# RocketFlash/EmbeddingNet

Hardware: AMD Instinct MI355X
Metric: images/sec training (ResNet18, 224², triplet batch-hard) @ 1/2/4/8 GPU (higher is better)
Workload: dtype f32; 1 GPU; resnet18 224x224x3 synthetic U[0,1), 107-class P x K sampling, local batch 32x4=128 (139 resident batches cycled), E=256, margin 0.5, mining 'hardest' per local batch, radam, fp32 tensors (conv products on 16-bit MFMA from operand splits, fp32 accumulate: 3x3 stride-1 convs and their weight gradients, and the ResNets' other convs where both operands' ranges are known: two fp16 pieces + a per-tenso; global_batch=128, parallelism=dp1, active_triplets_min=192, dead_steps=0, resident_batches=139, step_mode=eager, mining=hardest

## Files before the change

embeddingnet_amd/csrc/conv.hip:

```cpp
#include "gemm_engine.h"
#include "conv_geom.h"
#include "../../include/embnet.h"
#include <stdlib.h>

namespace embnet {

struct InputTransform { const float* scale; const float* shift; int act; };
__device__ __forceinline__ float4 transform4(float4 v, bool ok, const float4& sc, const float4& sh, int act) {
  float4 z = make_float4(fmaf(v.x, sc.x, sh.x), fmaf(v.y, sc.y, sh.y), fmaf(v.z, sc.z, sh.z), fmaf(v.w, sc.w, sh.w));
  if (act == 1) {
    z = make_float4(fmaxf(z.x, 0.f), fmaxf(z.y, 0.f), fmaxf(z.z, 0.f), fmaxf(z.w, 0.f));
  } else if (act == 2) {
    z = make_float4(act_apply(2, z.x), act_apply(2, z.y), act_apply(2, z.z), act_apply(2, z.w));
  }
  return ok ? z : make_float4(0.f, 0.f, 0.f, 0.f);
}


template <int ROWS, bool VEC, bool TF = false>
struct LoadConvFwdA {
  using Tile = TileKC<ROWS>;
  static constexpr bool CAN_INTERLEAVE = VEC && !TF;
  Buf buf; int H, W, C, Kg; FastDiv dC, dS; int tid;
  unsigned base[Tile::PASSES]; int ih0[Tile::PASSES], iw0[Tile::PASSES];
// ... 356 lines not shown
        d.x += o.x; d.y += o.y; d.z += o.z; d.w += o.w;
      }
      const float4 o = red[2][threadIdx.x + s * qpb];
      float4& d = red[2][threadIdx.x];
      d.x = fmaxf(d.x, o.x); d.y = fmaxf(d.y, o.y); d.z = fmaxf(d.z, o.z); d.w = fmaxf(d.w, o.w);
    }
    __syncthreads();
  }
  if (rr == 0 && col < cols) {
    const long prow = (long)(tile / tiles_n) * (bm / wtm) + band, P = stats_rows;
    const float4 s1 = red[0][threadIdx.x], s2 = red[1][threadIdx.x];
    float* d1 = stats + (long)col * P + prow;
    float* d2 = d1 + (long)cols * P;
    d1[0] = s1.x; d1[P] = s1.y; d1[2 * P] = s1.z; d1[3 * P] = s1.w;
    d2[0] = s2.x; d2[P] = s2.y; d2[2 * P] = s2.z; d2[3 * P] = s2.w;
    if (bsum.x && bsum.kinds == 3) {
      const float4 s3 = red[2][threadIdx.x];
      float* d3 = d2 + (long)cols * P;
      d3[0] = s3.x; d3[P] = s3.y; d3[2 * P] = s3.z; d3[3 * P] = s3.w;
    }
  }
}

template <class G, bool VEC, bool TF, bool H = false>
__device__ __forceinline__ void conv_fwd_body(const ConvFwdParams& p) {
  using TA = TileKC<G::BM>;
  using TB = TileKM<G::BN>;
  __shared__ __attribute__((aligned(16))) float smem[SMEM_FLOATS<G, TA, TB>];
  prio_hi();
  const int M = p.g.N * p.g.OH * p.g.OW, Kg = p.g.R * p.g.S * p.g.C;
  const int tiles_n = (p.g.K + G::BN - 1) / G::BN;
  int id, k0, k1; float* part;
  tail_decode<G>(p.tail, blockIdx.x, (Kg + BK - 1) / BK, id, k0, k1, part);
  const int m0 = (id / tiles_n) * G::BM, n0 = (id % tiles_n) * G::BN;
  stamp(0);
  LoadConvFwdA<G::BM, VEC, TF> la; la.init(p.x, p.g, m0, threadIdx.x, p.tf);
  LoadRowsKM<G::BN, VEC> lb; lb.init(p.w, p.g.K, p.g.K, Kg, n0, threadIdx.x);
  f32x16 acc[G::TM][G::TN];
  stamp(2);
  if constexpr (H) {
    const float2 sa = range_scale(p.rg.a), sb = range_scale(p.rg.b);
    conv_mainloop<G, TA, TB, decltype(la), decltype(lb), true>(la, lb, k0, k1, smem, acc, (int)blockIdx.x >= p.fair_from, true, sa.x, sb.x);
    scale_acc<G>(acc, sa.y, sb.y);
  } else {
    conv_mainloop<G, TA, TB>(la, lb, k0, k1, smem, acc, (int)blockIdx.x >= p.fair_from);
  }
  stamp(4);
  if (part) { store_partial<G>(acc, smem, part); stamp(5); return; }
  if (VEC) {
    float4 s1 = make_float4(0.f, 0.f, 0.f, 0.f), s2 = s1;
    constexpr int NJ = EpiIdx<G>::NJ;
    const int ecol = n0 + epi_col<G>();
    const bool cok = ecol < p.g.K;
    float4 bv = make_float4(0.f, 0.f, 0.f, 0.f);
    if (p.bias && cok) bv = *reinterpret_cast<const float4*>(p.bias + ecol);
    float4 res[G::TM][NJ];
    if (p.residual) {
#pragma unroll
      for (int im = 0; im < G::TM; ++im)
#pragma unroll
        for (int j = 0; j < NJ; ++j)
          res[im][j] = *reinterpret_cast<const float4*>(p.residual + (long)min(m0 + epi_row<G>(im, j), M - 1) * p.g.K + (cok ? ecol : 0));
// ... 33 lines not shown
      }
    }
    stamp(5);
    return;
  }
  for_each_acc<G>(acc, [&](int r, int c, float v) {
    const int row = m0 + r, col = n0 + c;
    if (row < M && col < p.g.K) {
      if (p.bias) v += p.bias[col];
      if (p.relu) v = fmaxf(v, 0.f);
      if (p.residual) v += p.residual[(long)row * p.g.K + col];
      p.y[(long)row * p.g.K + col] = v;
    }
  });
}

template <class G, bool VEC>
__global__ __launch_bounds__(256, VEC ? CONV_OCC<G> : 1) void conv_fwd_kernel(ConvFwdParams p) { conv_fwd_body<G, VEC, false>(p); }
template <class G, bool VEC>
__global__ __launch_bounds__(256, CONV_OCC<G>) void conv_fwd_tf_kernel(ConvFwdParams p) { conv_fwd_body<G, true, true>(p); }
template <class G>
__global__ __launch_bounds__(256, CONV_OCC_H<G>) void conv_fwd_h_kernel(ConvFwdParams p) { conv_fwd_body<G, true, false, true>(p); }

struct ConvDgradParams { const float* dy; const float* w; float* dx; ConvGeom g; DgradClass cls[MAX_CLASSES]; SplitTail tail; int accumulate; const float* add_src; int fair_from; BnSums bn; Ranges rg; };

template <class G, bool VEC, bool H = false>
__device__ __forceinline__ void conv_dgrad_body(const ConvDgradParams& p) {
  using TA = TileKC<G::BM>;
  using TB = TileKC<G::BN>;
  __shared__ __attribute__((aligned(16))) float smem[SMEM_FLOATS<G, TA, TB>];
  prio_hi();
  const DgradClass& cg = p.cls[blockIdx.y];
  const int M = p.g.N * cg.Hc * cg.Wc, Kg = cg.nR * cg.nS * p.g.K;
  const int tiles_n = (p.g.C + G::BN - 1) / G::BN;
  int id, k0, k1; float* part;
  tail_decode<G>(p.tail, blockIdx.x, (Kg + BK - 1) / BK, id, k0, k1, part);
  const int m0 = (id / tiles_n) * G::BM, n0 = (id % tiles_n) * G::BN;
  if (m0 >= M) return;
  if (Kg == 0 && p.accumulate && p.add_src == p.dx) return;
  stamp(0);
  LoadConvDgradA<G::BM, VEC> la; la.init(p.dy, p.g, cg, m0, threadIdx.x);
  LoadConvDgradB<G::BN, VEC> lb; lb.init(p.w, p.g, cg, n0, threadIdx.x);
  f32x16 acc[G::TM][G::TN];
  stamp(2);
  if constexpr (H) {
    const float2 sa = range_scale(p.rg.a), sb = range_scale(p.rg.b);
    conv_mainloop<G, TA, TB, decltype(la), decltype(lb), true>(la, lb, k0, k1, smem, acc, (int)(blockIdx.y * gridDim.x + blockIdx.x) >= p.fair_from,
                                                               true, sa.x, sb.x);
    scale_acc<G>(acc, sa.y, sb.y);
  } else {
    conv_mainloop<G, TA, TB>(la, lb, k0, k1, smem, acc, (int)(blockIdx.y * gridDim.x + blockIdx.x) >= p.fair_from);
  }
  stamp(4);
  if (part) { store_partial<G>(acc, smem, part); stamp(5); return; }
  const int st = p.g.stride;
  if ((p.g.C & 3) == 0) {
    constexpr int NJ = EpiIdx<G>::NJ;
    const int ecol = n0 + epi_col<G>();
    const bool cok = ecol < p.g.C;
    long base[G::TM][NJ];
    float4 res[G::TM][NJ];
    const bool bnon = p.bn.x != nullptr;
    const float* pre = bnon ? p.bn.x : p.add_src;
#pragma unroll
    for (int im = 0; im < G::TM; ++im)
#pragma unroll
      for (int j = 0; j < NJ; ++j) {
        uint32_t n, rem, hc, wc;
        cg.dHWc.divmod((uint32_t)min(m0 + epi_row<G>(im, j), M - 1), n, rem); cg.dWc.divmod(rem, hc, wc);
        base[im][j] = (((long)n * p.g.H + cg.hoff + st * (int)hc) * p.g.W + cg.woff + st * (int)wc) * p.g.C;
        if (p.accumulate || bnon) res[im][j] = *reinterpret_cast<const float4*>(pre + base[im][j] + (cok ? ecol : 0));
      }
// ... 38 lines not shown
          d3[0] = s3.x; d3[P] = s3.y; d3[2 * P] = s3.z; d3[3 * P] = s3.w;
        }
      }
    }
    stamp(5);
    return;
  }
  int last_r = -1; long row_base = 0;
  for_each_acc<G>(acc, [&](int r, int c, float v) {
    const int row = m0 + r, col = n0 + c;
    if (r != last_r) {
      last_r = r;
      uint32_t n, rem, hc, wc;
      cg.dHWc.divmod((uint32_t)min(row, M - 1), n, rem); cg.dWc.divmod(rem, hc, wc);
      row_base = (((long)n * p.g.H + cg.hoff + st * (int)hc) * p.g.W + cg.woff + st * (int)wc) * p.g.C;
    }
    if (row < M && col < p.g.C) p.dx[row_base + col] = p.accumulate ? p.add_src[row_base + col] + v : v;
  });
}
template <class G, bool VEC>
__global__ __launch_bounds__(256, VEC ? CONV_OCC<G> : 1) void conv_dgrad_kernel(ConvDgradParams p) { conv_dgrad_body<G, VEC>(p); }
template <class G>
__global__ __launch_bounds__(256, CONV_OCC_H<G>) void conv_dgrad_h_kernel(ConvDgradParams p) { conv_dgrad_body<G, true, true>(p); }

struct ConvWgradParams { const float* x; const float* dy; float* out; ConvGeom g; int kt_per_split, splits; InputTransform tf; int fair_from; Ranges rg; };

template <class G, bool VA, bool VB, bool TF, bool H = false>
__device__ __forceinline__ void conv_wgrad_body(const ConvWgradParams& p) {
  using TA = TileKM<G::BM>;
  using TB = TileKM<G::BN>;
  __shared__ __attribute__((aligned(16))) float smem[SMEM_FLOATS<G, TA, TB>];
  prio_hi();
  const int M = p.g.R * p.g.S * p.g.C, Kg = p.g.N * p.g.OH * p.g.OW;
  const int tiles_n = (p.g.K + G::BN - 1) / G::BN;
  const int tiles = ((M + G::BM - 1) / G::BM) * tiles_n;
  const int split = blockIdx.x / tiles, tile = blockIdx.x % tiles;
  if (split >= p.splits) return;
  const int m0 = (tile / tiles_n) * G::BM, n0 = (tile % tiles_n) * G::BN;
  const int kt_total = (Kg + BK - 1) / BK;
  const int kt0 = split * p.kt_per_split, kt1 = min(kt0 + p.kt_per_split, kt_total);
  stamp(0);
  LoadConvWgradA<G::BM, VA, TF> la; la.init(p.x, p.g, m0, threadIdx.x, p.tf);
  LoadRowsKM<G::BN, VB> lb; lb.init(p.dy, p.g.K, p.g.K, Kg, n0, threadIdx.x);
  f32x16 acc[G::TM][G::TN];
  stamp(2);
  if constexpr (H) {
// ... 296 lines not shown

extern "C" size_t embnet_conv2d_fwd_workspace_bytes(int n, int c, int r, int s, int k, int oh, int ow) {
  if (n <= 0 || c <= 0 || r <= 0 || s <= 0 || k <= 0 || oh <= 0 || ow <= 0 || ((c | k) & 3)) return 0;
  const long M = (long)n * oh * ow;
  const int tile = pick_tile(M, k, false, (long)r * s * c);
  SplitTail t; size_t need;
  plan_tail((long)cdiv(M, TILE_BM[tile]) * cdiv(k, TILE_BN[tile]), cdiv((long)r * s * c, BK), TILE_BM[tile], TILE_BN[tile],
            0, t, &need);
  return need;
}

extern "C" int embnet_conv2d_fwd_stats_rows(int n, int c, int r, int s, int k, int oh, int ow) {
  if (n <= 0 || c <= 0 || r <= 0 || s <= 0 || k <= 0 || oh <= 0 || ow <= 0 || ((c | k) & 3)) return 0;
  const long M = (long)n * oh * ow;
  if (r == 1 && s == 1 && thin_gemm_applies(c, k)) return thin_gemm_stats_rows(M, k);
  const int tile = pick_tile(M, k, false, (long)r * s * c);
  return cdiv(M, TILE_BM[tile]) * (TILE_BM[tile] / TILE_WTM[tile]);
}

static int conv2d_fwd_impl(const float* x, const float* w, const float* bias, float* y, int n, int h,
                           int wd, int c, int r, int s, int k, int stride, int pad_t, int pad_l, int oh,
                           int ow, int relu, const float* residual, const float* in_scale,
                           const float* in_shift, int in_act, float* stats, void* workspace,
                           size_t workspace_bytes, void* stream, const Ranges rg) {
  const bool ranged = ranges_ok(rg);
  EMBNET_CHECK_ARG(x && w && y, "conv2d_fwd: null pointer");
  EMBNET_CHECK_ARG(!in_scale == !in_shift, "conv2d_fwd: in_scale and in_shift go together");
  EMBNET_CHECK_ARG(aligned16(y) && aligned16(workspace) && aligned16(residual),
                   "conv2d_fwd: output, residual and workspace must be 16-byte aligned");
  ConvFwdParams p{x, w, bias, y, {}, relu, {}, residual};
  if (int rc = make_geom(p.g, n, h, wd, c, r, s, k, stride, pad_t, pad_l, oh, ow, "conv2d_fwd")) return rc;
  const long M = (long)n * oh * ow;
  hipStream_t st = (hipStream_t)stream;
  if (r == 1 && s == 1 && thin_gemm_applies(c, k)) {
    const bool can = pad_t == 0 && pad_l == 0 && !in_scale && aligned16(x) && aligned16(w) && aligned16(bias) && aligned16(stats);
    if (can) return launch_thin_gemm(x, w, 0, M, c, k, y, stats, bias, relu, residual, stride, n, h, wd, oh, ow, st);
    EMBNET_CHECK_ARG(!stats, "conv2d_fwd: epilogue statistics of a thin 1x1 conv go with pad 0 and no input transform");
  }
  const bool vec = (c & 3) == 0 && (k & 3) == 0 && aligned16(x) && aligned16(w) && (!bias || aligned16(bias));
  const bool hform = ranged && vec && !in_scale;
  const int tile = pick_tile(M, k, false, (long)r * s * c);
  const long tiles = (long)cdiv(M, TILE_BM[tile]) * cdiv(k, TILE_BN[tile]);
  EMBNET_CHECK_ARG(!in_scale || (vec && aligned16(in_scale) && aligned16(in_shift)),
                   "conv2d_fwd: the fused input transform needs channel counts that are multiples of 4 and aligned pointers");
  EMBNET_CHECK_ARG(!stats || (vec && aligned16(stats)),
                   "conv2d_fwd: epilogue statistics need channel counts that are multiples of 4 (see conv2d_fwd_stats_rows)");
  p.tf = InputTransform{in_scale, in_shift, in_act};
  p.stats = stats;
  p.stats_rows = cdiv(M, TILE_BM[tile]) * (TILE_BM[tile] / TILE_WTM[tile]);
  plan_tail(tiles, cdiv((long)r * s * c, BK), TILE_BM[tile], TILE_BN[tile], (vec && workspace) ? workspace_bytes : 0, p.tail);
  p.tail.ws = (float*)workspace;
  const int grid = p.tail.n_full + (int)(tiles - p.tail.n_full) * p.tail.parts;
  p.fair_from = fair_from(grid, tile, false);
  const double flop = 2.0 * M * k * r * s * c;
  p.rg = rg;
  {
    EMBNET_TRACE_FLOP(hform ? conv_h_kernel_name("conv_fwd_h_kernel", "ConvFwdParams", tile) :
                      conv_kernel_name(in_scale ? "conv_fwd_tf_kernel" : "conv_fwd_kernel", "ConvFwdParams", tile,
                                       (vec || in_scale) ? "true" : "false"), flop,
                      4.0 * ((double)n * h * wd * c + (double)r * s * c * k + (double)M * k * (residual ? 2 : 1)), st);
    if (hform) for_tile<false>(tile, [&](auto g) { conv_fwd_h_kernel<decltype(g)><<<grid, 256, 0, st>>>(p); });
    else if (in_scale) for_tile<false>(tile, [&](auto g) { conv_fwd_tf_kernel<decltype(g), true><<<grid, 256, 0, st>>>(p); });
    else if (vec) for_tile<false>(tile, [&](auto g) { conv_fwd_kernel<decltype(g), true><<<grid, 256, 0, st>>>(p); });
    else for_tile<false>(tile, [&](auto g) { conv_fwd_kernel<decltype(g), false><<<grid, 256, 0, st>>>(p); });
  }
  if (p.tail.parts > 1)
    launch_tail_fixup(p.tail.ws, p.tail.parts, TILE_BM[tile], TILE_BN[tile], TILE_WTM[tile], p.tail.n_full, (int)(tiles - p.tail.n_full),
                      cdiv(k, TILE_BN[tile]), M, k, bias, relu, residual, y, stats, p.stats_rows, NO_BN_SUMS, st);
  return check_launch("conv2d_fwd");
}
extern "C" int embnet_conv2d_fwd_f32(const float* x, const float* w, const float* bias, float* y, int n, int h,
                                     int wd, int c, int r, int s, int k, int stride, int pad_t, int pad_l, int oh,
                                     int ow, int relu, const float* residual, const float* in_scale,
                                     const float* in_shift, int in_act, float* stats, void* workspace,
                                     size_t workspace_bytes, void* stream) {
  return conv2d_fwd_impl(x, w, bias, y, n, h, wd, c, r, s, k, stride, pad_t, pad_l, oh, ow, relu, residual, in_scale, in_shift, in_act,
                         stats, workspace, workspace_bytes, stream, take_ranges());
}
extern "C" int embnet_conv2d_fwd_f32_ex(const float* x, const float* w, const float* bias, float* y, int n, int h,
                                        int wd, int c, int r, int s, int k, int stride, int pad_t, int pad_l, int oh,
                                        int ow, int relu, const float* residual, const float* in_scale,
                                        const float* in_shift, int in_act, float* stats, void* workspace,
                                        size_t workspace_bytes, const uint32_t* x_range, const uint32_t* w_range, void* stream) {
  (void)take_ranges();
  return conv2d_fwd_impl(x, w, bias, y, n, h, wd, c, r, s, k, stride, pad_t, pad_l, oh, ow, relu, residual, in_scale, in_shift, in_act,
                         stats, workspace, workspace_bytes, stream, Ranges{x_range, w_range});
}

extern "C" size_t embnet_conv2d_dgrad_workspace_bytes(int n, int h, int wd, int c, int r, int s, int k, int stride) {
  if (n <= 0 || h <= 0 || wd <= 0 || c <= 0 || r <= 0 || s <= 0 || k <= 0 || stride != 1 || ((c | k) & 3)) return 0;
  const long M = (long)n * h * wd;
  const int tile = pick_tile(M, c, false, (long)r * s * k);
  SplitTail t; size_t need;
  plan_tail((long)cdiv(M, TILE_BM[tile]) * cdiv(c, TILE_BN[tile]), cdiv((long)r * s * k, BK), TILE_BM[tile], TILE_BN[tile],
            0, t, &need);
  return need;
}

static int conv2d_dgrad_impl(const float* dy, const float* w, float* dx, int n, int h, int wd, int c,
                             int r, int s, int k, int stride, int pad_t, int pad_l, int oh, int ow,
                             int accumulate, const float* dx_add, void* workspace, size_t workspace_bytes,
                             void* stream, const BnSums bn, const Ranges rg) {
  const bool ranged = ranges_ok(rg);
  EMBNET_CHECK_ARG(dy && w && dx, "conv2d_dgrad: null pointer");
  EMBNET_CHECK_ARG(aligned16(dx) && aligned16(workspace), "conv2d_dgrad: output and workspace must be 16-byte aligned");
  EMBNET_CHECK_ARG(!(accumulate && dx_add), "conv2d_dgrad: accumulate (into dx) or dx_add (another tensor), not both");
  EMBNET_CHECK_ARG(aligned16(dx_add), "conv2d_dgrad: dx_add must be 16-byte aligned");
  ConvDgradParams p{dy, w, dx, {}, {}, {}, (accumulate != 0 || dx_add) ? 1 : 0, dx_add ? dx_add : dx};
  p.bn = bn;
  if (int rc = make_geom(p.g, n, h, wd, c, r, s, k, stride, pad_t, pad_l, oh, ow, "conv2d_dgrad")) return rc;
  if (r == 1 && s == 1 && stride == 1 && pad_t == 0 && pad_l == 0 && !accumulate && !dx_add && !bn.partial && aligned16(dy) &&
      aligned16(w) && thin_gemm_applies(k, c))
    return launch_thin_gemm(dy, w, 1, (long)n * h * wd, k, c, dx, nullptr, nullptr, 0, nullptr, 1, n, h, wd, h, wd, (hipStream_t)stream);
  EMBNET_CHECK_ARG(stride * stride <= MAX_CLASSES, "conv2d_dgrad: stride %d > 3 unsupported", stride);
  long max_m = 0;
  for (int ph = 0; ph < stride; ++ph)
    for (int pw = 0; pw < stride; ++pw) {
      DgradClass& cg = p.cls[ph * stride + pw];
      cg.r0 = ph; cg.s0 = pw;
      cg.hoff = ((ph - pad_t) % stride + stride) % stride; cg.woff = ((pw - pad_l) % stride + stride) % stride;
      cg.Hc = cg.hoff < h ? (h - cg.hoff + stride - 1) / stride : 0;
      cg.Wc = cg.woff < wd ? (wd - cg.woff + stride - 1) / stride : 0;
      cg.nR = ph < r ? (r - ph + stride - 1) / stride : 0;
      cg.nS = pw < s ? (s - pw + stride - 1) / stride : 0;
      cg.hb = (cg.hoff + pad_t - ph) / stride; cg.wb = (cg.woff + pad_l - pw) / stride;
      cg.dHWc = FastDiv::make(cg.Hc * cg.Wc > 0 ? cg.Hc * cg.Wc : 1);
      cg.dWc = FastDiv::make(cg.Wc > 0 ? cg.Wc : 1);
      cg.dnS = FastDiv::make(cg.nS > 0 ? cg.nS : 1);
      const long m = (long)n * cg.Hc * cg.Wc;
      if (m > max_m) max_m = m;
    }
  hipStream_t st = (hipStream_t)stream;
  const int tile = pick_tile(max_m * stride * stride, c, stride > 1, (long)r * s * k);
  const long tiles = (long)cdiv(max_m, TILE_BM[tile]) * cdiv(c, TILE_BN[tile]);
  const bool vec = (k & 3) == 0 && aligned16(dy) && aligned16(w);
  const bool can_split = vec && stride == 1 && (c & 3) == 0 && workspace;
  plan_tail(tiles, cdiv((long)p.cls[0].nR * p.cls[0].nS * k, BK), TILE_BM[tile], TILE_BN[tile],
            can_split ? workspace_bytes : 0, p.tail);
  p.tail.ws = (float*)workspace;
  const dim3 grid(p.tail.n_full + (int)(tiles - p.tail.n_full) * p.tail.parts, stride * stride);
  p.fair_from = fair_from((long)grid.x * grid.y, tile, false);
  const bool hform = ranged && vec;
  p.rg = rg;
  {
    EMBNET_TRACE_FLOP(hform ? conv_h_kernel_name("conv_dgrad_h_kernel", "ConvDgradParams", tile) :
                      conv_kernel_name("conv_dgrad_kernel", "ConvDgradParams", tile, vec ? "true" : "false"),
                      2.0 * n * oh * ow * (double)k * r * s * c,
                      4.0 * ((double)n * oh * ow * k + (double)r * s * c * k + (double)n * h * wd * c * (p.accumulate ? 2 : 1)), st);
    if (hform) for_tile<false>(tile, [&](auto g) { conv_dgrad_h_kernel<decltype(g)><<<grid, 256, 0, st>>>(p); });
    else if (vec) for_tile<false>(tile, [&](auto g) { conv_dgrad_kernel<decltype(g), true><<<grid, 256, 0, st>>>(p); });
    else for_tile<false>(tile, [&](auto g) { conv_dgrad_kernel<decltype(g), false><<<grid, 256, 0, st>>>(p); });
  }
  if (p.tail.parts > 1)
    launch_tail_fixup(p.tail.ws, p.tail.parts, TILE_BM[tile], TILE_BN[tile], TILE_WTM[tile], p.tail.n_full, (int)(tiles - p.tail.n_full),
                      cdiv(c, TILE_BN[tile]), max_m, c, nullptr, 0, p.accumulate ? p.add_src : nullptr, dx, nullptr, 0, p.bn, st);
  return check_launch("conv2d_dgrad");
}

extern "C" int embnet_conv2d_dgrad_f32(const float* dy, const float* w, float* dx, int n, int h, int wd, int c,
                                       int r, int s, int k, int stride, int pad_t, int pad_l, int oh, int ow,
                                       int accumulate, const float* dx_add, void* workspace, size_t workspace_bytes,
                                       void* stream) {
  return conv2d_dgrad_impl(dy, w, dx, n, h, wd, c, r, s, k, stride, pad_t, pad_l, oh, ow, accumulate, dx_add, workspace,
                           workspace_bytes, stream, NO_BN_SUMS, take_ranges());
}
extern "C" int embnet_conv2d_dgrad_f32_ex(const float* dy, const float* w, float* dx, int n, int h, int wd, int c,
                                          int r, int s, int k, int stride, int pad_t, int pad_l, int oh, int ow,
                                          int accumulate, const float* dx_add, void* workspace, size_t workspace_bytes,
                                          const uint32_t* dy_range, const uint32_t* w_range, void* stream) {
  (void)take_ranges();
  return conv2d_dgrad_impl(dy, w, dx, n, h, wd, c, r, s, k, stride, pad_t, pad_l, oh, ow, accumulate, dx_add, workspace,
                           workspace_bytes, stream, NO_BN_SUMS, Ranges{dy_range, w_range});
}

extern "C" int embnet_conv2d_dgrad_bnsums_rows(int n, int h, int wd, int c, int r, int s, int k, int stride) {
  if (n <= 0 || h <= 0 || wd <= 0 || c <= 0 || r <= 0 || s <= 0 || k <= 0 || stride != 1 || ((c | k) & 3)) return 0;
  const long M = (long)n * h * wd;
  const int tile = pick_tile(M, c, false, (long)r * s * k);
  return cdiv(M, TILE_BM[tile]) * (TILE_BM[tile] / TILE_WTM[tile]);
// ... 10 lines not shown
  EMBNET_CHECK_ARG(aligned16(bn_x) && aligned16(bn_scale) && aligned16(bn_shift) && aligned16(bn_mean) && aligned16(bn_rstd) &&
                   aligned16(dy) && aligned16(w), "conv2d_dgrad_bnsums: operands must be 16-byte aligned");
  EMBNET_CHECK_ARG(bn_act >= 0 && bn_act <= 2, "conv2d_dgrad_bnsums: activation code %d", bn_act);
  return conv2d_dgrad_impl(dy, w, dx, n, h, wd, c, r, s, k, stride, pad_t, pad_l, oh, ow, 0, nullptr, workspace, workspace_bytes,
                           stream, BnSums{bn_x, bn_scale, bn_shift, bn_mean, bn_rstd, bn_act, bn_partial, bn_rows, kinds}, rg);
}
extern "C" int embnet_conv2d_dgrad_bnsums_f32(const float* dy, const float* w, float* dx, int n, int h, int wd, int c, int r,
                                              int s, int k, int stride, int pad_t, int pad_l, int oh, int ow,
                                              const float* bn_x, const float* bn_scale, const float* bn_shift,
                                              const float* bn_mean, const float* bn_rstd, int bn_act, float* bn_partial,
                                              int bn_rows, void* workspace, size_t workspace_bytes, void* stream) {
  return conv2d_dgrad_bnsums_impl(dy, w, dx, n, h, wd, c, r, s, k, stride, pad_t, pad_l, oh, ow, bn_x, bn_scale, bn_shift, bn_mean,
                                  bn_rstd, bn_act, bn_partial, bn_rows, workspace, workspace_bytes, stream, take_ranges());
}
extern "C" int embnet_conv2d_dgrad_bnsums_f32_ex(const float* dy, const float* w, float* dx, int n, int h, int wd, int c, int r,
                                                 int s, int k, int stride, int pad_t, int pad_l, int oh, int ow,
                                                 const float* bn_x, const float* bn_scale, const float* bn_shift,
                                                 const float* bn_mean, const float* bn_rstd, int bn_act, float* bn_partial,
                                                 int bn_rows, void* workspace, size_t workspace_bytes,
                                                 const uint32_t* dy_range, const uint32_t* w_range, void* stream) {
  (void)take_ranges();
  return conv2d_dgrad_bnsums_impl(dy, w, dx, n, h, wd, c, r, s, k, stride, pad_t, pad_l, oh, ow, bn_x, bn_scale, bn_shift, bn_mean,
                                  bn_rstd, bn_act, bn_partial, bn_rows, workspace, workspace_bytes, stream, Ranges{dy_range, w_range}, 3);
}

static void wgrad_plan(int rows, int k, long kg, int& tile, int& splits, int& kt_per_split, bool one_by_one = false) {
  if (one_by_one && thin_wgrad_applies(rows, k)) {
    tile = -1; splits = thin_wgrad_splits(kg, rows, k); kt_per_split = 0;
    return;
  }
  tile = (rows <= 64 && k > 32) ? 3 : (k <= 32 ? 2 : (k <= 64 ? 1 : 0));
  if (tile == 1 && rows % 192 == 0 && rows % 128 != 0) tile = 4;
  const int forced_tile = (int)env_long("EMBNET_WGRAD_TILE", -1);
  if (forced_tile >= 0) tile = forced_tile;
  const long tiles = (long)cdiv(rows, TILE_BM[tile]) * cdiv(k, TILE_BN[tile]);
  const int kt_total = cdiv(kg, BK);
#if EMBNET_CONV_SPLIT
  long target = tiles >= 100 ? 1024 : (tiles <= 2 ? 768 : 512);
#else
  long target = tiles >= 100 ? 2048 : (tiles >= 30 ? 1536 : 768);
#endif
  const long forced_blocks = env_long("EMBNET_WGRAD_BLOCKS", 0);
  if (forced_blocks > 0) target = forced_blocks;
#if EMBNET_CONV_SPLIT
  long want = target / tiles;
#else
// ... 122 lines not shown
                                       size_t workspace_bytes, int n, int h, int wd, int c, int r, int s, int k,
                                       int stride, int pad_t, int pad_l, int oh, int ow, const float* in_scale, const float* in_shift, int in_act,
        const uint32_t* x_range, const uint32_t* dy_range, void* stream) {
  (void)take_ranges();
  return wgrad_impl(x, dy, dw, workspace, workspace_bytes, n, h, wd, c, r, s, k, stride, pad_t, pad_l, oh, ow, in_scale, in_shift, in_act,
                    stream, true, false, Ranges{x_range, dy_range});
}
extern "C" int embnet_conv2d_wgrad_reduce_f32(const float* x, const float* dy, float* dw, void* workspace,
                                       size_t workspace_bytes, int n, int h, int wd, int c, int r, int s, int k,
                                       int stride, int pad_t, int pad_l, int oh, int ow, const float* in_scale, const float* in_shift, int in_act,
        void* stream) {
  return wgrad_impl(x, dy, dw, workspace, workspace_bytes, n, h, wd, c, r, s, k, stride, pad_t, pad_l, oh, ow, in_scale, in_shift, in_act,
                    stream, false, true, take_ranges());
}

extern "C" const char* embnet_conv2d_kernel_name(int kind, int n, int h, int wd, int c, int r, int s, int k,
                                                 int oh, int ow) {
  if (kind == 0)
    return conv_kernel_name("conv_fwd_kernel", "ConvFwdParams", pick_tile((long)n * oh * ow, k, false, (long)r * s * c),
                            ((c | k) & 3) == 0 ? "true" : "false");
  if (kind == 1)
    return conv_kernel_name("conv_dgrad_kernel", "ConvDgradParams", pick_tile((long)n * h * wd, c, oh < h, (long)r * s * k),
                            (k & 3) == 0 ? "true" : "false");
  if (kind != 2) return "";
  int tile, sp, kt;
  wgrad_plan(r * s * c, k, (long)n * oh * ow, tile, sp, kt, r == 1 && s == 1);
  if (tile < 0) return "embnet::thinw::thin_wgrad_kernel";
  return conv_kernel_name("conv_wgrad_kernel", "ConvWgradParams", tile,
                          (k & 3) ? "false, false" : ((c & 3) ? "false, true" : "true, true"));
}
```

embeddingnet_amd/layers.py:

```python
import contextlib
import math
import os as _os

import torch
from torch import nn

from . import _lib
from ._lib import check, ptr, stream


def env_switch(var, default):
    return {"0": False, "1": True}.get(_os.environ.get(var), default)


@contextlib.contextmanager
def switches(**values):
    old = {name: globals()[name][0] for name in values}
    try:
        for name, v in values.items():
            globals()[name][0] = v
        yield
    finally:
        for name, v in old.items():
            globals()[name][0] = v
# ... 658 lines not shown
                        _rptr(dy_range), _rptr(w_range) if dy_range is not None else None, stream()))
                    BN_SUMS.put(dx.data_ptr(), (partial, rows, bn_x.data_ptr(), dx.detach()), 8, "oldest")
                else:
                    _gather_dgrad(lib, dz, w, dx, n, h, wd, c, r, s, k, stride, pt, pl, oh, ow, dy_range, w_range, 0, dskip)
        if need_dw:
            conv_wgrad(lib, x, dz, dw, w, n, h, wd, c, r, s, k, stride, pt, pl, oh, ow, in_scale, in_shift, ctx.in_act,
                       ctx.x_planes, dy_planes, dy_range, ctx.x_range)
            dw = _done(dw, dw_note)
        if want_db:
            db, db_note = _sink(ctx.bias_ref)
            _colsum(dz.view(-1, k), out=db)
            db = _done(db, db_note)
        if dskip is not None and dx is None and ctx.needs_input_grad[0]:
            dx = dskip
        if ctx.has_res and dy_only_planes:
            raise _lib.EmbnetError("conv2d backward: a conv with a fused Add received its gradient as planes only; the Add's other "
                                   "branch needs the fp32 gradient (BatchNormalization(owns_input=True) behind conv(residual=...))")
        return dx, dw, db, None, None, (dy if ctx.has_res else None), None, None, None, None, None, None, None, None, None


class _ConvPairFn(torch.autograd.Function):

    @staticmethod
    def forward(ctx, x, w1, geom1, w2, geom2, in_stats, in_act, out_stats1, planes=None, w_ranges=None, x_range=None):
        w_ranges = tuple(w_ranges) if (w_ranges is not None and in_stats is None and x_range is not None) else (None, None)
        x, w1, w2 = _c(x), _c(w1), _c(w2)
        lib = _lib.lib()
        n, h, wd, c = x.shape
        in_scale, in_shift = _in_affine(in_stats)
        ys = []
        for w, geom, st in ((w1, geom1, out_stats1), (w2, geom2, None)):
            r, s, c2, k = w.shape
            if c2 != c:
                raise _lib.EmbnetError(f"conv2d: input has {c} channels, kernel expects {c2}")
            stride, pt, pl, oh, ow = geom
            y = torch.empty((n, oh, ow, k), device=x.device, dtype=torch.float32)
            if planes is not None and w is w1:
                ws = workspace(lib.embnet_conv2d_patch_workspace_bytes(n, c, r, s, k, oh, ow), x.device)
                check(lib.embnet_conv2d_patch_f32(ptr(planes), ptr(weight_planes(w, 0)), None, ptr(y), n, h, wd, c, r, s, k,
                                                  pt, pl, oh, ow, 0, None, ptr(st), ptr(ws), ws.numel() * 4, stream()))
            else:
                _gather_fwd(lib, x, w, None, y, n, h, wd, c, r, s, k, stride, pt, pl, oh, ow, x_range, w_ranges[0 if w is w1 else 1],
                            st, 0, None, in_scale, in_shift, in_act)
            ys.append(y)
        ctx.patch = planes is not None
        ctx.w_ranges = (w_ranges[0] if planes is None else None, w_ranges[1])
        ctx.x_range = x_range
        ctx.x_planes = planes
        ctx.geoms, ctx.in_act = (geom1, geom2), int(in_act)
        ctx.save_for_backward(x, w1, w2, in_stats)
        return ys[0], ys[1]

    @staticmethod
    def backward(ctx, dy1, dy2):
        x, w1, w2, in_stats = ctx.saved_tensors
        lib = _lib.lib()
        n, h, wd, c = x.shape
        in_scale, in_shift = _in_affine(in_stats)
        dx = torch.empty_like(x) if ctx.needs_input_grad[0] else None
        dws, first = [], True
        for w, geom, dy, need_dw in ((w1, ctx.geoms[0], dy1, ctx.needs_input_grad[1]),
                                     (w2, ctx.geoms[1], dy2, ctx.needs_input_grad[3])):
            if dy is None:
                dws.append(None)
                continue
            if not _is_placeholder(dy):
                dy = _c(dy)
            r, s, _, k = w.shape
            stride, pt, pl, oh, ow = geom
            dy_planes = _take_dy_planes(dy) if (ctx.patch and w is w1) else None
            if _is_placeholder(dy) and dy_planes is None:
                raise _lib.EmbnetError("conv_pair backward: the gradient exists only as planes and they are gone (DY_PLANES)")
            w_range = ctx.w_ranges[0 if w is w1 else 1]
            dy_range = _take_dy_range(dy) if (w_range is not None and not _is_placeholder(dy)) else None
            if dx is not None:
                if dy_planes is not None and first and patch_ok(n, oh, ow, k, r, s, c, 1, h, wd):
                    _patch_dgrad(dy_planes, w, dx, n, h, wd, c, r, s, k, pt, pl, oh, ow, None)
                else:
                    _gather_dgrad(lib, dy, w, dx, n, h, wd, c, r, s, k, stride, pt, pl, oh, ow, dy_range, w_range, 0 if first else 1)
                first = False
            dw = None
            if need_dw:
                dw, note = _sink(w)
                conv_wgrad(lib, x, dy, dw, w, n, h, wd, c, r, s, k, stride, pt, pl, oh, ow, in_scale, in_shift, ctx.in_act,
                           ctx.x_planes if w is w1 else None, dy_planes, dy_range, ctx.x_range if w_range is not None else None)
                dw = _done(dw, note)
            dws.append(dw)
        if dx is not None and first:
            dx.zero_()
        return dx, dws[0], None, dws[1], None, None, None, None, None, None, None


def conv_pair(x, conv1, conv2, emit_stats=False):
    if conv1.bias is not None or conv2.bias is not None or conv1.relu or conv2.relu:
        return conv1(x, emit_stats=emit_stats), conv2(x)
    in_stats, in_act = None, 0
    if isinstance(x, Deferred):
        if any(cv.kernel.shape[2] % 4 or cv.kernel.shape[3] % 4 for cv in (conv1, conv2)):
# ... 1422 lines not shown
```

include/embnet.h:

```cpp
#ifndef EMBNET_H
#define EMBNET_H

#include <stddef.h>
#include <stdint.h>

#ifdef __cplusplus
extern "C" {
#endif

#define EMBNET_ABI_VERSION 22

enum {
  EMBNET_MINE_SEMIHARD = 0,
  EMBNET_MINE_HARDEST = 1,
  EMBNET_MINE_RANDOM_HARD = 2,
  EMBNET_MINE_BATCH_HARD = 3
};

int embnet_abi_version(void);
const char* embnet_last_error(void);

int embnet_trace_enable(int on);
int embnet_trace_reset(void);
int embnet_trace_count(void);
// ... 107 lines not shown
int embnet_conv2d_ranges(const uint32_t* a, const uint32_t* b);
int embnet_conv2d_fwd_f32_ex(const float* x, const float* w, const float* bias, float* y, int n, int h, int wd, int c,
                             int r, int s, int k, int stride, int pad_t, int pad_l, int oh, int ow, int relu,
                             const float* residual, const float* in_scale, const float* in_shift, int in_act,
                             float* stats, void* workspace, size_t workspace_bytes, const uint32_t* x_range,
                             const uint32_t* w_range, void* stream);
int embnet_conv2d_dgrad_f32_ex(const float* dy, const float* w, float* dx, int n, int h, int wd, int c, int r, int s,
                               int k, int stride, int pad_t, int pad_l, int oh, int ow, int accumulate, const float* dx_add,
                               void* workspace, size_t workspace_bytes, const uint32_t* dy_range, const uint32_t* w_range,
                               void* stream);
int embnet_conv2d_dgrad_bnsums_f32_ex(const float* dy, const float* w, float* dx, int n, int h, int wd, int c, int r, int s,
                                      int k, int stride, int pad_t, int pad_l, int oh, int ow, const float* bn_x,
                                      const float* bn_scale, const float* bn_shift, const float* bn_mean, const float* bn_rstd,
                                      int bn_act, float* bn_partial, int bn_rows, void* workspace, size_t workspace_bytes,
                                      const uint32_t* dy_range, const uint32_t* w_range, void* stream);
int embnet_conv2d_wgrad_f32_ex(const float* x, const float* dy, float* dw, void* workspace, size_t workspace_bytes,
                               int n, int h, int wd, int c, int r, int s, int k, int stride, int pad_t, int pad_l,
                               int oh, int ow, const float* in_scale, const float* in_shift, int in_act,
                               const uint32_t* x_range, const uint32_t* dy_range, void* stream);
int embnet_conv2d_wgrad_slabs_f32_ex(const float* x, const float* dy, float* dw, void* workspace, size_t workspace_bytes,
                                     int n, int h, int wd, int c, int r, int s, int k, int stride, int pad_t, int pad_l,
                                     int oh, int ow, const float* in_scale, const float* in_shift, int in_act,
                                     const uint32_t* x_range, const uint32_t* dy_range, void* stream);

const char* embnet_conv2d_kernel_name(int kind, int n, int h, int wd, int c, int r, int s, int k, int oh, int ow);

int embnet_conv1x1_thin_supported(int red, int ncols);

int embnet_conv2d_patch_supported(int n, int c, int r, int s, int k, int stride, int oh, int ow);
size_t embnet_conv2d_patch_workspace_bytes(int n, int c, int r, int s, int k, int oh, int ow);
int embnet_conv2d_patch_stats_rows(int n, int oh, int ow);
int embnet_conv2d_patch_f32(const void* x_planes, const void* w_planes, const float* bias, float* y, int n, int h, int wd, int c,
                            int r, int s, int k, int pad_t, int pad_l, int oh, int ow, int relu, const float* residual,
                            float* stats, void* workspace, size_t workspace_bytes, void* stream);
int embnet_conv2d_stem_supported(int n, int h, int wd, int c, int r, int s, int k, int stride, int pad_t, int pad_l, int oh, int ow);
int embnet_conv2d_stem_stats_rows(int n, int oh, int ow);
int embnet_conv2d_stem_f32(const float* x, const float* w, float* y, int n, int h, int wd, int pad_t, int pad_l, int oh, int ow,
                           float* stats, const uint32_t* x_range, const uint32_t* w_range, void* stream);
int embnet_conv2d_planes1x1_f32(const void* x_planes, const void* w_planes, const float* bias, float* y, int n, int h, int wd, int c,
                                int k, int stride, int oh, int ow, int relu, const float* residual, float* stats,
                                void* workspace, size_t workspace_bytes, void* stream);
int embnet_conv2d_dma1x1_supported(int n, int h, int wd, int c, int k, int stride, int oh, int ow);
int embnet_conv2d_dma1x1_f32(const float* x, const void* wp, const float* bias, float* y, int n, int h, int wd, int c, int k,
                             int stride, int oh, int ow, int relu, const float* residual, float* stats, const uint32_t* x_range,
                             void* workspace, size_t workspace_bytes, void* stream);
int embnet_conv2d_patch_bnsums_f32(const void* x_planes, const void* w_planes, float* y, int n, int h, int wd, int c, int r, int s,
// ... 224 lines not shown
```

Baseline: 16390 images/sec.

## Fuse strided 3x3 conv with its 1x1 downsample conv in forward and dgrad

Adds paired kernels for the ResNet downsample blocks. In forward, the tile that starts at k0==0 first runs the 1x1 shortcut conv over the centre-tap slice of the shared input tiles, writes y2, and then runs the 3x3 conv. In dgrad, the 1x1 conv's contribution is added into the accumulators of the matching stride class, so the two dx passes and the extra accumulate launch collapse into one kernel. This saves launches and input re-reads at the cost of more work per block in some tiles, which can cause load imbalance, plus extra register pressure from a second accumulator set.

```diff
diff --git a/embeddingnet_amd/csrc/conv.hip b/embeddingnet_amd/csrc/conv.hip
--- a/embeddingnet_amd/csrc/conv.hip
+++ b/embeddingnet_amd/csrc/conv.hip
@@ -402,8 +402,18 @@
   }
 }
 
-template <class G, bool VEC, bool TF, bool H = false>
-__device__ __forceinline__ void conv_fwd_body(const ConvFwdParams& p) {
+struct PairFwd { const float* w2; float* y2; const uint32_t* w2_range; int kc0, kc1; };
+template <int ROWS>
+struct LoadRowsKMFrom {
+  using Tile = TileKM<ROWS>;
+  static constexpr bool CAN_INTERLEAVE = false;
+  LoadRowsKM<ROWS, true> l; int shift;
+  __device__ __forceinline__ void fix(float4 (&)[Tile::PASSES]) const {}
+  __device__ __forceinline__ void load(int kt, float4 (&r)[Tile::PASSES]) const { l.load(kt - shift, r); }
+};
+
+template <class G, bool VEC, bool TF, bool H = false, bool PAIR = false>
+__device__ __forceinline__ void conv_fwd_body(const ConvFwdParams& p, const PairFwd* q = nullptr) {
   using TA = TileKC<G::BM>;
   using TB = TileKM<G::BN>;
   __shared__ __attribute__((aligned(16))) float smem[SMEM_FLOATS<G, TA, TB>];
@@ -418,6 +428,19 @@
   LoadRowsKM<G::BN, VEC> lb; lb.init(p.w, p.g.K, p.g.K, Kg, n0, threadIdx.x);
   f32x16 acc[G::TM][G::TN];
   stamp(2);
+  if constexpr (PAIR) {
+    if (k0 == 0) {
+      LoadRowsKMFrom<G::BN> lb2; lb2.l.init(q->w2, p.g.K, p.g.K, p.g.C, n0, threadIdx.x); lb2.shift = q->kc0;
+      const float2 sa = range_scale(p.rg.a), sb2 = range_scale(q->w2_range);
+      conv_mainloop<G, TA, TB, decltype(la), decltype(lb2), true>(la, lb2, q->kc0, q->kc1, smem, acc, (int)blockIdx.x >= p.fair_from, true, sa.x, sb2.x);
+      scale_acc<G>(acc, sa.y, sb2.y);
+      for_each_acc_row4<G>(acc, smem, [&](int r, int c, float4 v) {
+        const int row = m0 + r, col = n0 + c;
+        if (row < M && col < p.g.K) *reinterpret_cast<float4*>(q->y2 + (long)row * p.g.K + col) = v;
+      });
+      prio_hi();
+    }
+  }
   if constexpr (H) {
     const float2 sa = range_scale(p.rg.a), sb = range_scale(p.rg.b);
     conv_mainloop<G, TA, TB, decltype(la), decltype(lb), true>(la, lb, k0, k1, smem, acc, (int)blockIdx.x >= p.fair_from, true, sa.x, sb.x);
@@ -497,10 +520,15 @@
 template <class G>
 __global__ __launch_bounds__(256, CONV_OCC_H<G>) void conv_fwd_h_kernel(ConvFwdParams p) { conv_fwd_body<G, true, false, true>(p); }
 
+template <class G>
+__global__ __launch_bounds__(256, CONV_OCC_H<G>) void conv_pair_fwd_h_kernel(ConvFwdParams p, PairFwd q) { conv_fwd_body<G, true, false, true, true>(p, &q); }
+
 struct ConvDgradParams { const float* dy; const float* w; float* dx; ConvGeom g; DgradClass cls[MAX_CLASSES]; SplitTail tail; int accumulate; const float* add_src; int fair_from; BnSums bn; Ranges rg; };
 
-template <class G, bool VEC, bool H = false>
-__device__ __forceinline__ void conv_dgrad_body(const ConvDgradParams& p) {
+struct PairDgrad { const float* dy2; const float* w2; ConvGeom g2; DgradClass cls2; int cls; Ranges rg2; };
+
+template <class G, bool VEC, bool H = false, bool PAIR = false>
+__device__ __forceinline__ void conv_dgrad_body(const ConvDgradParams& p, const PairDgrad* q = nullptr) {
   using TA = TileKC<G::BM>;
   using TB = TileKC<G::BN>;
   __shared__ __attribute__((aligned(16))) float smem[SMEM_FLOATS<G, TA, TB>];
@@ -523,6 +551,21 @@
     conv_mainloop<G, TA, TB, decltype(la), decltype(lb), true>(la, lb, k0, k1, smem, acc, (int)(blockIdx.y * gridDim.x + blockIdx.x) >= p.fair_from,
                                                                true, sa.x, sb.x);
     scale_acc<G>(acc, sa.y, sb.y);
+    if constexpr (PAIR) {
+      if ((int)blockIdx.y == q->cls) {
+        LoadConvDgradA<G::BM, VEC> la2; la2.init(q->dy2, q->g2, q->cls2, m0, threadIdx.x);
+        LoadConvDgradB<G::BN, VEC> lb2; lb2.init(q->w2, q->g2, q->cls2, n0, threadIdx.x);
+        f32x16 acc2[G::TM][G::TN];
+        const float2 sa2 = range_scale(q->rg2.a), sb2 = range_scale(q->rg2.b);
+        conv_mainloop<G, TA, TB, decltype(la2), decltype(lb2), true>(la2, lb2, 0, (q->cls2.nR * q->cls2.nS * q->g2.K + BK - 1) / BK, smem, acc2,
+                                                                     (int)(blockIdx.y * gridDim.x + blockIdx.x) >= p.fair_from, true, sa2.x, sb2.x);
+        scale_acc<G>(acc2, sa2.y, sb2.y);
+#pragma unroll
+        for (int i = 0; i < G::TM; ++i)
+#pragma unroll
+          for (int j = 0; j < G::TN; ++j) acc[i][j] += acc2[i][j];
+      }
+    }
   } else {
     conv_mainloop<G, TA, TB>(la, lb, k0, k1, smem, acc, (int)(blockIdx.y * gridDim.x + blockIdx.x) >= p.fair_from);
   }
@@ -607,6 +650,9 @@
 __global__ __launch_bounds__(256, VEC ? CONV_OCC<G> : 1) void conv_dgrad_kernel(ConvDgradParams p) { conv_dgrad_body<G, VEC>(p); }
 template <class G>
 __global__ __launch_bounds__(256, CONV_OCC_H<G>) void conv_dgrad_h_kernel(ConvDgradParams p) { conv_dgrad_body<G, true, true>(p); }
+
+template <class G>
+__global__ __launch_bounds__(256, CONV_OCC_H<G>) void conv_pair_dgrad_h_kernel(ConvDgradParams p, PairDgrad q) { conv_dgrad_body<G, true, true, true>(p, &q); }
 
 struct ConvWgradParams { const float* x; const float* dy; float* out; ConvGeom g; int kt_per_split, splits; InputTransform tf; int fair_from; Ranges rg; };
 
@@ -949,7 +995,7 @@
                            int wd, int c, int r, int s, int k, int stride, int pad_t, int pad_l, int oh,
                            int ow, int relu, const float* residual, const float* in_scale,
                            const float* in_shift, int in_act, float* stats, void* workspace,
-                           size_t workspace_bytes, void* stream, const Ranges rg) {
+                           size_t workspace_bytes, void* stream, const Ranges rg, const PairFwd* pair = nullptr) {
   const bool ranged = ranges_ok(rg);
   EMBNET_CHECK_ARG(x && w && y, "conv2d_fwd: null pointer");
   EMBNET_CHECK_ARG(!in_scale == !in_shift, "conv2d_fwd: in_scale and in_shift go together");
@@ -966,6 +1012,7 @@
   }
   const bool vec = (c & 3) == 0 && (k & 3) == 0 && aligned16(x) && aligned16(w) && (!bias || aligned16(bias));
   const bool hform = ranged && vec && !in_scale;
+  EMBNET_CHECK_ARG(!pair || hform, "conv2d_pair_fwd: needs the ranges of x, w1 and w2 and 16-byte aligned operands");
   const int tile = pick_tile(M, k, false, (long)r * s * c);
   const long tiles = (long)cdiv(M, TILE_BM[tile]) * cdiv(k, TILE_BN[tile]);
   EMBNET_CHECK_ARG(!in_scale || (vec && aligned16(in_scale) && aligned16(in_shift)),
@@ -981,7 +1028,7 @@
   p.fair_from = fair_from(grid, tile, false);
   const double flop = 2.0 * M * k * r * s * c;
   p.rg = rg;
-  {
+  if (!pair) {
     EMBNET_TRACE_FLOP(hform ? conv_h_kernel_name("conv_fwd_h_kernel", "ConvFwdParams", tile) :
                       conv_kernel_name(in_scale ? "conv_fwd_tf_kernel" : "conv_fwd_kernel", "ConvFwdParams", tile,
                                        (vec || in_scale) ? "true" : "false"), flop,
@@ -990,11 +1037,16 @@
     else if (in_scale) for_tile<false>(tile, [&](auto g) { conv_fwd_tf_kernel<decltype(g), true><<<grid, 256, 0, st>>>(p); });
     else if (vec) for_tile<false>(tile, [&](auto g) { conv_fwd_kernel<decltype(g), true><<<grid, 256, 0, st>>>(p); });
     else for_tile<false>(tile, [&](auto g) { conv_fwd_kernel<decltype(g), false><<<grid, 256, 0, st>>>(p); });
+  } else {
+    const PairFwd q = *pair;
+    EMBNET_TRACE_FLOP(conv_h_kernel_name("conv_pair_fwd_h_kernel", "ConvFwdParams, embnet::PairFwd", tile), flop + 2.0 * M * k * c,
+                      4.0 * ((double)n * h * wd * c + (double)(r * s + 1) * c * k + 2.0 * M * k), st);
+    for_tile<false>(tile, [&](auto g) { conv_pair_fwd_h_kernel<decltype(g)><<<grid, 256, 0, st>>>(p, q); });
   }
   if (p.tail.parts > 1)
     launch_tail_fixup(p.tail.ws, p.tail.parts, TILE_BM[tile], TILE_BN[tile], TILE_WTM[tile], p.tail.n_full, (int)(tiles - p.tail.n_full),
                       cdiv(k, TILE_BN[tile]), M, k, bias, relu, residual, y, stats, p.stats_rows, NO_BN_SUMS, st);
-  return check_launch("conv2d_fwd");
+  return check_launch(pair ? "conv2d_pair_fwd" : "conv2d_fwd");
 }
 extern "C" int embnet_conv2d_fwd_f32(const float* x, const float* w, const float* bias, float* y, int n, int h,
                                      int wd, int c, int r, int s, int k, int stride, int pad_t, int pad_l, int oh,
@@ -1027,7 +1079,7 @@
 static int conv2d_dgrad_impl(const float* dy, const float* w, float* dx, int n, int h, int wd, int c,
                              int r, int s, int k, int stride, int pad_t, int pad_l, int oh, int ow,
                              int accumulate, const float* dx_add, void* workspace, size_t workspace_bytes,
-                             void* stream, const BnSums bn, const Ranges rg) {
+                             void* stream, const BnSums bn, const Ranges rg, PairDgrad* pair = nullptr) {
   const bool ranged = ranges_ok(rg);
   EMBNET_CHECK_ARG(dy && w && dx, "conv2d_dgrad: null pointer");
   EMBNET_CHECK_ARG(aligned16(dx) && aligned16(workspace), "conv2d_dgrad: output and workspace must be 16-byte aligned");
@@ -1069,7 +1121,7 @@
   p.fair_from = fair_from((long)grid.x * grid.y, tile, false);
   const bool hform = ranged && vec;
   p.rg = rg;
-  {
+  if (!pair) {
     EMBNET_TRACE_FLOP(hform ? conv_h_kernel_name("conv_dgrad_h_kernel", "ConvDgradParams", tile) :
                       conv_kernel_name("conv_dgrad_kernel", "ConvDgradParams", tile, vec ? "true" : "false"),
                       2.0 * n * oh * ow * (double)k * r * s * c,
@@ -1077,11 +1129,35 @@
     if (hform) for_tile<false>(tile, [&](auto g) { conv_dgrad_h_kernel<decltype(g)><<<grid, 256, 0, st>>>(p); });
     else if (vec) for_tile<false>(tile, [&](auto g) { conv_dgrad_kernel<decltype(g), true><<<grid, 256, 0, st>>>(p); });
     else for_tile<false>(tile, [&](auto g) { conv_dgrad_kernel<decltype(g), false><<<grid, 256, 0, st>>>(p); });
+  } else {
+    const ConvGeom& g2 = pair->g2;
+    EMBNET_CHECK_ARG(hform && ranges_ok(pair->rg2) && (g2.K & 3) == 0 && (c & 3) == 0 && aligned16(pair->dy2) && aligned16(pair->w2),
+                     "conv2d_pair_dgrad: needs the ranges of dy1, w1, dy2 and w2 and 16-byte aligned operands");
+    DgradClass& c2 = pair->cls2;
+    c2.r0 = 0; c2.s0 = 0;
+    c2.hoff = ((-g2.pad_t) % stride + stride) % stride; c2.woff = ((-g2.pad_l) % stride + stride) % stride;
+    c2.Hc = c2.hoff < h ? (h - c2.hoff + stride - 1) / stride : 0;
+    c2.Wc = c2.woff < wd ? (wd - c2.woff + stride - 1) / stride : 0;
+    c2.nR = 1; c2.nS = 1;
+    c2.hb = (c2.hoff + g2.pad_t) / stride; c2.wb = (c2.woff + g2.pad_l) / stride;
+    c2.dHWc = FastDiv::make(c2.Hc * c2.Wc > 0 ? c2.Hc * c2.Wc : 1);
+    c2.dWc = FastDiv::make(c2.Wc > 0 ? c2.Wc : 1);
+    c2.dnS = FastDiv::make(1);
+    pair->cls = -1;
+    for (int i = 0; i < stride * stride; ++i)
+      if (p.cls[i].hoff == c2.hoff && p.cls[i].woff == c2.woff) pair->cls = i;
+    EMBNET_CHECK_ARG(pair->cls >= 0 && p.cls[pair->cls].Hc == c2.Hc && p.cls[pair->cls].Wc == c2.Wc && p.tail.parts == 1,
+                     "conv2d_pair_dgrad: the pair is not fusable (embnet_conv2d_pair_fusable)");
+    EMBNET_TRACE_FLOP(conv_h_kernel_name("conv_pair_dgrad_h_kernel", "ConvDgradParams, embnet::PairDgrad", tile),
+                      2.0 * n * oh * ow * ((double)k * r * s * c + (double)g2.K * c),
+                      4.0 * ((double)n * oh * ow * (k + g2.K) + (double)r * s * c * k + (double)c * g2.K + (double)n * h * wd * c), st);
+    const PairDgrad q = *pair;
+    for_tile<false>(tile, [&](auto g) { conv_pair_dgrad_h_kernel<decltype(g)><<<grid, 256, 0, st>>>(p, q); });
   }
   if (p.tail.parts > 1)
     launch_tail_fixup(p.tail.ws, p.tail.parts, TILE_BM[tile], TILE_BN[tile], TILE_WTM[tile], p.tail.n_full, (int)(tiles - p.tail.n_full),
                       cdiv(c, TILE_BN[tile]), max_m, c, nullptr, 0, p.accumulate ? p.add_src : nullptr, dx, nullptr, 0, p.bn, st);
-  return check_launch("conv2d_dgrad");
+  return check_launch(pair ? "conv2d_pair_dgrad" : "conv2d_dgrad");
 }
 
 extern "C" int embnet_conv2d_dgrad_f32(const float* dy, const float* w, float* dx, int n, int h, int wd, int c,
@@ -1138,6 +1214,51 @@
   (void)take_ranges();
   return conv2d_dgrad_bnsums_impl(dy, w, dx, n, h, wd, c, r, s, k, stride, pad_t, pad_l, oh, ow, bn_x, bn_scale, bn_shift, bn_mean,
                                   bn_rstd, bn_act, bn_partial, bn_rows, workspace, workspace_bytes, stream, Ranges{dy_range, w_range}, 3);
+}
+
+extern "C" int embnet_conv2d_pair_fusable(int c, int r1, int s1, int k1, int stride1, int pad_t1, int pad_l1, int oh1, int ow1,
+                                          int r2, int s2, int k2, int stride2, int pad_t2, int pad_l2, int oh2, int ow2) {
+  if (!EMBNET_CONV_SPLIT || c <= 0 || k1 <= 0 || k2 <= 0 || oh1 <= 0 || ow1 <= 0) return 0;
+  if (r2 != 1 || s2 != 1 || stride1 != stride2 || oh1 != oh2 || ow1 != ow2) return 0;
+  const int rc = pad_t1 - pad_t2, sc = pad_l1 - pad_l2;
+  if (pad_t2 < 0 || pad_l2 < 0 || rc < 0 || rc >= r1 || sc < 0 || sc >= s1) return 0;
+  if ((c % 32) || (k1 & 3) || (k2 & 3)) return 0;
+  return r1 == 3 && s1 == 3 && stride1 == 2 && k2 == k1;
+}
+extern "C" int embnet_conv2d_pair_tap_tile(int c, int r1, int s1, int pad_t1, int pad_l1, int pad_t2, int pad_l2) {
+  const int rc = pad_t1 - pad_t2, sc = pad_l1 - pad_l2;
+  if (c <= 0 || (c % 32) || rc < 0 || rc >= r1 || sc < 0 || sc >= s1) return -1;
+  return (rc * s1 + sc) * (c / BK);
+}
+extern "C" int embnet_conv2d_pair_fwd_f32_ex(const float* x, const float* w1, const float* w2, float* y1, float* y2, int n, int h,
+                                             int wd, int c, int r, int s, int k, int stride, int pad_t, int pad_l, int pad_t2,
+                                             int pad_l2, int oh, int ow, float* stats, void* workspace, size_t workspace_bytes,
+                                             const uint32_t* x_range, const uint32_t* w1_range, const uint32_t* w2_range,
+                                             void* stream) {
+  (void)take_ranges();
+  EMBNET_CHECK_ARG(w2 && y2 && aligned16(w2) && aligned16(y2) && w2_range && !(reinterpret_cast<uintptr_t>(w2_range) & 3),
+                   "conv2d_pair_fwd: w2, y2 (16-byte aligned) and w2's range");
+  EMBNET_CHECK_ARG(embnet_conv2d_pair_fusable(c, r, s, k, stride, pad_t, pad_l, oh, ow, 1, 1, k, stride, pad_t2, pad_l2, oh, ow),
+                   "conv2d_pair_fwd: the pair is not fusable (embnet_conv2d_pair_fusable)");
+  EMBNET_CHECK_ARG((oh - 1) * stride - pad_t2 < h && (ow - 1) * stride - pad_l2 < wd, "conv2d_pair_fwd: the 1x1 conv reaches outside the input");
+  PairFwd q{w2, y2, w2_range, 0, 0};
+  q.kc0 = embnet_conv2d_pair_tap_tile(c, r, s, pad_t, pad_l, pad_t2, pad_l2);
+  q.kc1 = q.kc0 + c / BK;
+  return conv2d_fwd_impl(x, w1, nullptr, y1, n, h, wd, c, r, s, k, stride, pad_t, pad_l, oh, ow, 0, nullptr, nullptr, nullptr, 0,
+                         stats, workspace, workspace_bytes, stream, Ranges{x_range, w1_range}, &q);
+}
+extern "C" int embnet_conv2d_pair_dgrad_f32_ex(const float* dy1, const float* w1, const float* dy2, const float* w2, float* dx, int n,
+                                               int h, int wd, int c, int r, int s, int k, int stride, int pad_t, int pad_l, int pad_t2,
+                                               int pad_l2, int oh, int ow, const uint32_t* dy1_range, const uint32_t* w1_range,
+                                               const uint32_t* dy2_range, const uint32_t* w2_range, void* stream) {
+  (void)take_ranges();
+  EMBNET_CHECK_ARG(dy2 && w2, "conv2d_pair_dgrad: null pointer");
+  EMBNET_CHECK_ARG(embnet_conv2d_pair_fusable(c, r, s, k, stride, pad_t, pad_l, oh, ow, 1, 1, k, stride, pad_t2, pad_l2, oh, ow),
+                   "conv2d_pair_dgrad: the pair is not fusable (embnet_conv2d_pair_fusable)");
+  PairDgrad q{dy2, w2, {}, {}, -1, Ranges{dy2_range, w2_range}};
+  if (int rc = make_geom(q.g2, n, h, wd, c, 1, 1, k, stride, pad_t2, pad_l2, oh, ow, "conv2d_pair_dgrad")) return rc;
+  return conv2d_dgrad_impl(dy1, w1, dx, n, h, wd, c, r, s, k, stride, pad_t, pad_l, oh, ow, 0, nullptr, nullptr, 0, stream, NO_BN_SUMS,
+                           Ranges{dy1_range, w1_range}, &q);
 }
 
 static void wgrad_plan(int rows, int k, long kg, int& tile, int& splits, int& kt_per_split, bool one_by_one = false) {
@@ -1306,6 +1427,10 @@
   if (kind == 1)
     return conv_kernel_name("conv_dgrad_kernel", "ConvDgradParams", pick_tile((long)n * h * wd, c, oh < h, (long)r * s * k),
                             (k & 3) == 0 ? "true" : "false");
+  if (kind == 3)
+    return conv_h_kernel_name("conv_pair_fwd_h_kernel", "ConvFwdParams, embnet::PairFwd", pick_tile((long)n * oh * ow, k, false, (long)r * s * c));
+  if (kind == 4)
+    return conv_h_kernel_name("conv_pair_dgrad_h_kernel", "ConvDgradParams, embnet::PairDgrad", pick_tile((long)n * h * wd, c, oh < h, (long)r * s * k));
   if (kind != 2) return "";
   int tile, sp, kt;
   wgrad_plan(r * s * c, k, (long)n * oh * ow, tile, sp, kt, r == 1 && s == 1);
diff --git a/embeddingnet_amd/layers.py b/embeddingnet_amd/layers.py
--- a/embeddingnet_amd/layers.py
+++ b/embeddingnet_amd/layers.py
@@ -704,6 +704,12 @@
 class _ConvPairFn(torch.autograd.Function):
 
     @staticmethod
+    def _fusable(lib, c, w1, geom1, w2, geom2):
+        (r1, s1, _, k1), (r2, s2, _, k2) = w1.shape, w2.shape
+        return bool(lib.embnet_conv2d_pair_fusable(c, r1, s1, k1, geom1[0], geom1[1], geom1[2], geom1[3], geom1[4],
+                                                   r2, s2, k2, geom2[0], geom2[1], geom2[2], geom2[3], geom2[4]))
+
+    @staticmethod
     def forward(ctx, x, w1, geom1, w2, geom2, in_stats, in_act, out_stats1, planes=None, w_ranges=None, x_range=None):
         w_ranges = tuple(w_ranges) if (w_ranges is not None and in_stats is None and x_range is not None) else (None, None)
         x, w1, w2 = _c(x), _c(w1), _c(w2)
@@ -711,10 +717,20 @@
         n, h, wd, c = x.shape
         in_scale, in_shift = _in_affine(in_stats)
         ys = []
-        for w, geom, st in ((w1, geom1, out_stats1), (w2, geom2, None)):
+        if w1.shape[2] != c or w2.shape[2] != c:
+            raise _lib.EmbnetError(f"conv2d: input has {c} channels, kernels expect {w1.shape[2]} and {w2.shape[2]}")
+        fused = (planes is None and w_ranges[0] is not None and w_ranges[1] is not None
+                 and _ConvPairFn._fusable(lib, c, w1, geom1, w2, geom2))
+        if fused:
+            r, s, _, k = w1.shape
+            stride, pt, pl, oh, ow = geom1
+            ys = [torch.empty((n, oh, ow, k), device=x.device, dtype=torch.float32) for _ in range(2)]
+            ws = workspace(lib.embnet_conv2d_fwd_workspace_bytes(n, c, r, s, k, oh, ow), x.device)
+            check(lib.embnet_conv2d_pair_fwd_f32_ex(
+                ptr(x), ptr(w1), ptr(w2), ptr(ys[0]), ptr(ys[1]), n, h, wd, c, r, s, k, stride, pt, pl, geom2[1], geom2[2], oh, ow,
+                ptr(out_stats1), ptr(ws), ws.numel() * 4, _rptr(x_range), _rptr(w_ranges[0]), _rptr(w_ranges[1]), stream()))
+        for w, geom, st in ((w1, geom1, out_stats1), (w2, geom2, None)) if not fused else ():
             r, s, c2, k = w.shape
-            if c2 != c:
-                raise _lib.EmbnetError(f"conv2d: input has {c} channels, kernel expects {c2}")
             stride, pt, pl, oh, ow = geom
             y = torch.empty((n, oh, ow, k), device=x.device, dtype=torch.float32)
             if planes is not None and w is w1:
@@ -726,6 +742,7 @@
                             st, 0, None, in_scale, in_shift, in_act)
             ys.append(y)
         ctx.patch = planes is not None
+        ctx.fused = fused
         ctx.w_ranges = (w_ranges[0] if planes is None else None, w_ranges[1])
         ctx.x_range = x_range
         ctx.x_planes = planes
@@ -740,22 +757,37 @@
         n, h, wd, c = x.shape
         in_scale, in_shift = _in_affine(in_stats)
         dx = torch.empty_like(x) if ctx.needs_input_grad[0] else None
-        dws, first = [], True
+        dws, first, items = [], True, []
         for w, geom, dy, need_dw in ((w1, ctx.geoms[0], dy1, ctx.needs_input_grad[1]),
                                      (w2, ctx.geoms[1], dy2, ctx.needs_input_grad[3])):
             if dy is None:
-                dws.append(None)
+                items.append(None)
                 continue
             if not _is_placeholder(dy):
                 dy = _c(dy)
-            r, s, _, k = w.shape
-            stride, pt, pl, oh, ow = geom
             dy_planes = _take_dy_planes(dy) if (ctx.patch and w is w1) else None
             if _is_placeholder(dy) and dy_planes is None:
                 raise _lib.EmbnetError("conv_pair backward: the gradient exists only as planes and they are gone (DY_PLANES)")
             w_range = ctx.w_ranges[0 if w is w1 else 1]
             dy_range = _take_dy_range(dy) if (w_range is not None and not _is_placeholder(dy)) else None
-            if dx is not None:
+            items.append((w, geom, dy, need_dw, dy_planes, w_range, dy_range))
+        fused = ctx.fused and dx is not None and all(it is not None and it[6] is not None for it in items)
+        if fused:
+            (_, geom, g1, _, _, wr1, gr1), (_, geom2, g2, _, _, wr2, gr2) = items
+            r, s, _, k = w1.shape
+            stride, pt, pl, oh, ow = geom
+            check(lib.embnet_conv2d_pair_dgrad_f32_ex(
+                ptr(g1), ptr(w1), ptr(g2), ptr(w2), ptr(dx), n, h, wd, c, r, s, k, stride, pt, pl, geom2[1], geom2[2], oh, ow,
+                _rptr(gr1), _rptr(wr1), _rptr(gr2), _rptr(wr2), stream()))
+            first = False
+        for it in items:
+            if it is None:
+                dws.append(None)
+                continue
+            w, geom, dy, need_dw, dy_planes, w_range, dy_range = it
+            r, s, _, k = w.shape
+            stride, pt, pl, oh, ow = geom
+            if dx is not None and not fused:
                 if dy_planes is not None and first and patch_ok(n, oh, ow, k, r, s, c, 1, h, wd):
                     _patch_dgrad(dy_planes, w, dx, n, h, wd, c, r, s, k, pt, pl, oh, ow, None)
                 else:
diff --git a/include/embnet.h b/include/embnet.h
--- a/include/embnet.h
+++ b/include/embnet.h
@@ -153,6 +153,18 @@
                                      int n, int h, int wd, int c, int r, int s, int k, int stride, int pad_t, int pad_l,
                                      int oh, int ow, const float* in_scale, const float* in_shift, int in_act,
                                      const uint32_t* x_range, const uint32_t* dy_range, void* stream);
+
+int embnet_conv2d_pair_fusable(int c, int r1, int s1, int k1, int stride1, int pad_t1, int pad_l1, int oh1, int ow1,
+                               int r2, int s2, int k2, int stride2, int pad_t2, int pad_l2, int oh2, int ow2);
+int embnet_conv2d_pair_tap_tile(int c, int r1, int s1, int pad_t1, int pad_l1, int pad_t2, int pad_l2);
+int embnet_conv2d_pair_fwd_f32_ex(const float* x, const float* w1, const float* w2, float* y1, float* y2, int n, int h, int wd,
+                                  int c, int r, int s, int k, int stride, int pad_t, int pad_l, int pad_t2, int pad_l2, int oh,
+                                  int ow, float* stats, void* workspace, size_t workspace_bytes, const uint32_t* x_range,
+                                  const uint32_t* w1_range, const uint32_t* w2_range, void* stream);
+int embnet_conv2d_pair_dgrad_f32_ex(const float* dy1, const float* w1, const float* dy2, const float* w2, float* dx, int n, int h,
+                                    int wd, int c, int r, int s, int k, int stride, int pad_t, int pad_l, int pad_t2, int pad_l2,
+                                    int oh, int ow, const uint32_t* dy1_range, const uint32_t* w1_range,
+                                    const uint32_t* dy2_range, const uint32_t* w2_range, void* stream);
 
 const char* embnet_conv2d_kernel_name(int kind, int n, int h, int wd, int c, int r, int s, int k, int oh, int ow);
 
```

Measured after the change: 16480 images/sec (median of 6 runs). About the same (+0.6%).
